# addtt/ladder-vae-pytorch

Measured on AMD Instinct MI355X. Metric: training images/sec (ELBO step: fwd+bwd+Adamax), higher is better.
Workload: dtype f32; 1 GPU; CIFAR10-shaped 15-layer LVAE (BASELINE configs[2]): 32x32x3, zdims 32x15, 4 blocks/layer, 64 filters, gated+skip, DMoL-10, dropout 0.2, free bits 1.0; batch_per_gpu=256, global_batch=256, parallelism=dp1, hip_graph=True

## Files before the change

include/lvae_hip.h:

```cpp
#ifndef LVAE_HIP_H
#define LVAE_HIP_H

#include <stddef.h>
#include <stdint.h>

#ifdef __cplusplus
extern "C" {
#endif

#define LVAE_ABI_VERSION 17

#define LVAE_EINVAL (-1)
#define LVAE_EALIGN (-2)
#define LVAE_EWORKSPACE (-3)

enum { LVAE_STATS_BN_FWD = 0, LVAE_STATS_BN_BWD = 1 };
enum { LVAE_PREC_F32 = 0, LVAE_PREC_BF16 = 1 };
enum { LVAE_DT_F32 = 0, LVAE_DT_BF16 = 1 };
enum {
  LVAE_FORM_AUTO = 0,
  LVAE_FORM_F32_MFMA = 1,
  LVAE_FORM_SIX_PRODUCT = 2,
  LVAE_FORM_SIX_PRODUCT_DIRECT = 3
};
// ... 63 lines not shown
  LVAE_VARIANT_WINO_SIX = 4,
  LVAE_VARIANT_BF16_DIRECT = 5,
  LVAE_VARIANT_SIX_DIRECT = 6
};
int32_t lvae_conv2d_variant(const lvae_conv_desc* d);
int32_t lvae_conv2d_position_major(const lvae_conv_desc* d);
int32_t lvae_resblock_bf16_storage(const lvae_conv_desc* d);
int lvae_conv2d_bf16(const lvae_conv_desc* d, void* stream);
int32_t lvae_conv2d_stats_rows(const lvae_conv_desc* d);
int32_t lvae_conv2d_folds_bn_finalize(const lvae_conv_desc* d);
int32_t lvae_conv2d_stats_buffer_rows(const lvae_conv_desc* d);

size_t lvae_conv2d_prepare_entry_bytes(void);
int lvae_conv2d_prepare_entry(const lvae_conv_desc* d, void* entry);
int lvae_conv2d_prepare_weights(const void* entries, int32_t n, int32_t max_cout, void* stream);

int lvae_conv1x1_gate_f32(const lvae_conv_desc* d, const float* res, int32_t act, float* out, void* stream);
int32_t lvae_conv1x1_gate_stats_rows(const lvae_conv_desc* d);
enum {
  LVAE_GATE_PERSISTENT = 1,
  LVAE_GATE_SINGLE_SHOT = 2
};
int32_t lvae_conv1x1_gate_variant(const lvae_conv_desc* d);
int lvae_conv1x1_gate_bwd_f32(const lvae_conv_desc* d, const float* dout, const float* ab, int32_t act, float* dab,
                              void* stream);
int32_t lvae_conv1x1_gate_bwd_ok(const lvae_conv_desc* d);

typedef struct lvae_bn_apply {
  const float* parts;
  int32_t rows;
  int32_t act;
  int64_t M;
  const float* coef;
  const float* dh;
  const float* x;
  const float* add;
  float* dgamma;
  float* dbeta;
  float* out;
  int32_t dh_bf16;
  int32_t reserved_;
  const float* drop;
} lvae_bn_apply;
size_t lvae_conv1x1_gate_bwd_wgrad_workspace(const lvae_conv_desc* d);
int32_t lvae_conv1x1_gate_bwd_wgrad_apply_ok(const lvae_conv_desc* d);
int lvae_conv1x1_gate_bwd_wgrad_f32(const lvae_conv_desc* d, const float* dout, const float* ab, const float* y, int32_t act,
                                    float* dw, int64_t dw_sk, int64_t dw_sn, float* db, void* workspace, size_t workspace_bytes,
                                    const lvae_bn_apply* ap, void* stream);
int32_t lvae_conv1x1_gate_bwd_wgrad_recompute_ok(const lvae_conv_desc* d);
int lvae_conv1x1_gate_bwd_wgrad_recompute_f32(const lvae_conv_desc* d, const float* dout, const float* y, int32_t act, void* gate_ws,
                                              int64_t gate_ws_bytes, int32_t gate_ws_ready, const float* gate_w, int64_t gate_w_sk,
                                              int64_t gate_w_sn, const float* gate_bias, float* dw, int64_t dw_sk, int64_t dw_sn,
                                              float* db, void* workspace, size_t workspace_bytes, const lvae_bn_apply* ap, void* stream);

enum { LVAE_RB_PRO_AFFINE = 0, LVAE_RB_PRO_BN_APPLY = 1, LVAE_RB_PRO_GATE_BWD = 2 };
enum { LVAE_RB_EPI_PLAIN = 0, LVAE_RB_EPI_GATE = 1 };
typedef struct lvae_rb_ext {
  int32_t prologue, epilogue;
  const float* gate_w;
  int64_t gate_w_sk, gate_w_sn;
  void* gate_ws;
  int64_t gate_ws_bytes;
  int32_t gate_ws_ready;
  const float* gate_bias;
  int32_t act;
  const float* res;
  float* ab;
  float* out;
  float* out_stats;
  const float* out_stats_pivot;
  const float* dout;
  const float* ab_in;
  float* dab;
  const float* bwd_parts;
  int32_t bwd_rows;
  int32_t bwd_act;
  int64_t bwd_M;
  const float* bwd_coef;
  const float* bwd_x;
  float* dgamma;
  float* dbeta;
  const float* pro_drop;
  float* xt_out;
  const void* pf_ptr[2];
  int64_t pf_bytes[2];
  const float* ap_parts;
  int32_t ap_rows;
  int32_t ap_act;
  int64_t ap_M;
  const float* ap_coef;
  const float* ap_dh;
  const float* ap_x;
  const float* ap_add;
  float* ap_dgamma;
  float* ap_dbeta;
  float* ap_out;
} lvae_rb_ext;
size_t lvae_resblock_gate_workspace(const lvae_conv_desc* g);
int lvae_resblock_gate_prepare_entry(const lvae_conv_desc* g, void* entry);
int32_t lvae_resblock_conv_rows(const lvae_conv_desc* d);
int32_t lvae_resblock_conv_gate_rows(const lvae_conv_desc* d);
size_t lvae_resblock_conv_workspace(const lvae_conv_desc* d);
int lvae_resblock_conv_prepare_entry(const lvae_conv_desc* d, void* entry);
int lvae_resblock_conv_f32(const lvae_conv_desc* d, const lvae_rb_ext* ext, void* stream);

size_t lvae_conv2d_wgrad_workspace(const lvae_conv_desc* d);
// ... 257 lines not shown
```

ladder-vae-pytorch_amd/_C.py:

```python
import ctypes as C
import os

import torch

_HERE = os.path.dirname(os.path.abspath(__file__))
LIB_PATH = os.path.join(_HERE, 'liblvae_hip.so')

ACT = {None: 0, 'none': 0, 'elu': 1, 'relu': 2, 'leakyrelu': 3, 'selu': 4}
GATHER_CONV, GATHER_TRANSPOSED = 0, 1
PREC_F32, PREC_BF16 = 0, 1
DT_F32, DT_BF16 = 0, 1
VARIANT_DIRECT, VARIANT_POS, VARIANT_WINO_F32, VARIANT_WINO_SIX, VARIANT_BF16_DIRECT, VARIANT_SIX_DIRECT = 0, 2, 3, 4, 5, 6
GATE_PERSISTENT, GATE_SINGLE_SHOT = 1, 2
WGRAD_VARIANT_GENERIC, WGRAD_VARIANT_IMG, WGRAD_VARIANT_BF16, WGRAD_VARIANT_WINO, WGRAD_VARIANT_DIRECT_1X1, WGRAD_VARIANT_TILE, WGRAD_VARIANT_THIN = range(7)
FEED_U8, FEED_F32 = 0, 1
FORM_AUTO, FORM_F32_MFMA, FORM_SIX_PRODUCT, FORM_SIX_PRODUCT_DIRECT = 0, 1, 2, 3


class LvaeHipError(RuntimeError):
    pass


class ConvDesc(C.Structure):
    _fields_ = [
# ... 47 lines not shown


class LrScheduleStruct(C.Structure):
    _fields_ = [('base_lr', C.c_float), ('min_lr', C.c_float), ('gamma', C.c_float), ('kind', C.c_int32),
                ('warmup_steps', C.c_int64), ('decay_steps', C.c_int64)]


class GradGuardState(C.Structure):
    _fields_ = [('norm', C.c_float), ('scale', C.c_float), ('skip', C.c_int32), ('reserved_', C.c_int32), ('clipped', C.c_uint64),
                ('skipped', C.c_uint64)]


class CopyEntry(C.Structure):
    _fields_ = [('dst', C.c_void_p), ('src', C.c_void_p), ('n', C.c_int64)]


LR_KINDS = {'constant': 0, 'cosine': 1, 'linear': 2, 'step': 3, 'exp': 4}

RB_PRO_AFFINE, RB_PRO_BN_APPLY, RB_PRO_GATE_BWD = 0, 1, 2
RB_EPI_PLAIN, RB_EPI_GATE = 0, 1

ABI_VERSION = 17

_P, _I, _L, _F, _Z, _U = C.c_void_p, C.c_int32, C.c_int64, C.c_float, C.c_size_t, C.c_uint64

SIGNATURES = {
    'lvae_abi_version': (C.c_int, []),
    'lvae_last_error': (C.c_char_p, []),
    'lvae_conv2d_workspace': (_Z, [C.POINTER(ConvDesc)]),
    'lvae_conv2d_f32': (C.c_int, [C.POINTER(ConvDesc), _P]),
    'lvae_conv2d_bf16': (C.c_int, [C.POINTER(ConvDesc), _P]),
    'lvae_conv1x1_dgrad_cat_f32': (C.c_int, [C.POINTER(ConvDesc), _P, _I, _P]),
    'lvae_conv1x1_dgrad_cat_ok': (_I, [C.POINTER(ConvDesc), _I]),
    'lvae_conv2d_stats_rows': (_I, [C.POINTER(ConvDesc)]),
    'lvae_conv2d_variant': (_I, [C.POINTER(ConvDesc)]),
    'lvae_conv2d_position_major': (_I, [C.POINTER(ConvDesc)]),
    'lvae_resblock_bf16_storage': (_I, [C.POINTER(ConvDesc)]),
    'lvae_conv2d_folds_bn_finalize': (_I, [C.POINTER(ConvDesc)]),
    'lvae_conv2d_stats_buffer_rows': (_I, [C.POINTER(ConvDesc)]),
    'lvae_conv2d_prepare_entry_bytes': (_Z, []),
    'lvae_conv2d_prepare_entry': (C.c_int, [C.POINTER(ConvDesc), _P]),
    'lvae_conv2d_prepare_weights': (C.c_int, [_P, _I, _I, _P]),
    'lvae_conv1x1_gate_f32': (C.c_int, [C.POINTER(ConvDesc), _P, _I, _P, _P]),
    'lvae_conv1x1_gate_stats_rows': (_I, [C.POINTER(ConvDesc)]),
    'lvae_conv1x1_gate_variant': (_I, [C.POINTER(ConvDesc)]),
    'lvae_conv1x1_gate_bwd_f32': (C.c_int, [C.POINTER(ConvDesc), _P, _P, _I, _P, _P]),
    'lvae_conv1x1_gate_bwd_ok': (_I, [C.POINTER(ConvDesc)]),
    'lvae_conv1x1_gate_bwd_wgrad_workspace': (_Z, [C.POINTER(ConvDesc)]),
    'lvae_conv1x1_gate_bwd_wgrad_apply_ok': (_I, [C.POINTER(ConvDesc)]),
    'lvae_conv1x1_gate_bwd_wgrad_f32': (C.c_int, [C.POINTER(ConvDesc), _P, _P, _P, _I, _P, _L, _L, _P, _P, _Z, C.POINTER(BnApply), _P]),
    'lvae_conv1x1_gate_bwd_wgrad_recompute_ok': (_I, [C.POINTER(ConvDesc)]),
    'lvae_conv1x1_gate_bwd_wgrad_recompute_f32': (C.c_int, [C.POINTER(ConvDesc), _P, _P, _I, _P, _L, _I, _P, _L, _L, _P, _P, _L, _L, _P, _P, _Z,
                                                            C.POINTER(BnApply), _P]),
    'lvae_resblock_gate_workspace': (_Z, [C.POINTER(ConvDesc)]),
    'lvae_resblock_gate_prepare_entry': (C.c_int, [C.POINTER(ConvDesc), _P]),
    'lvae_resblock_conv_rows': (_I, [C.POINTER(ConvDesc)]),
    'lvae_resblock_conv_gate_rows': (_I, [C.POINTER(ConvDesc)]),
    'lvae_resblock_conv_workspace': (_Z, [C.POINTER(ConvDesc)]),
    'lvae_resblock_conv_prepare_entry': (C.c_int, [C.POINTER(ConvDesc), _P]),
    'lvae_resblock_conv_f32': (C.c_int, [C.POINTER(ConvDesc), C.POINTER(RbExt), _P]),
    'lvae_conv2d_wgrad_workspace': (_Z, [C.POINTER(ConvDesc)]),
    'lvae_conv2d_wgrad_f32': (C.c_int, [C.POINTER(ConvDesc), _P, _P, _P, _P, _Z, _P]),
    'lvae_conv2d_wgrad_bf16': (C.c_int, [C.POINTER(ConvDesc), _P, _P, _P, _P, _Z, _P]),
    'lvae_conv2d_wgrad_variant': (_I, [C.POINTER(ConvDesc)]),
    'lvae_conv2d_wgrad_apply_ok': (_I, [C.POINTER(ConvDesc)]),
    'lvae_conv2d_wgrad_apply_f32': (C.c_int, [C.POINTER(ConvDesc), C.POINTER(BnApply), _P, _P, _P, _Z, _P]),
    'lvae_conv2d_wgrad_pair_ok': (_I, [C.POINTER(ConvDesc), C.POINTER(ConvDesc)]),
    'lvae_conv2d_wgrad_pair_workspace': (_Z, [C.POINTER(ConvDesc), C.POINTER(ConvDesc)]),
    'lvae_conv2d_wgrad_pair_schedule': (_I, [C.POINTER(ConvDesc), C.POINTER(ConvDesc), C.POINTER(_I)]),
    'lvae_conv2d_wgrad_pair_f32': (C.c_int, [C.POINTER(ConvDesc), C.POINTER(BnApply), C.POINTER(ConvDesc), _P, _P, _P, _P, _P, _P, _Z, _P]),
    'lvae_conv2d_wgrad_shared_ok': (_I, [C.POINTER(ConvDesc), _P, _I]),
    'lvae_conv2d_wgrad_shared_workspace': (_Z, [C.POINTER(ConvDesc), _I]),
    'lvae_conv2d_wgrad_shared_schedule': (_I, [C.POINTER(ConvDesc), _P, _I, C.POINTER(_I)]),
    'lvae_conv2d_wgrad_shared_f32': (C.c_int, [C.POINTER(ConvDesc), _P, _P, _P, _I, _P, _Z, _P]),
    'lvae_conv2d_wgrad_grouped_workspace': (_Z, [C.POINTER(ConvDesc), _I]),
    'lvae_conv2d_wgrad_grouped_f32': (C.c_int, [C.POINTER(ConvDesc), _P, _P, _P, _I, _P, _Z, _P]),
    'lvae_conv2d_wgrad_grouped_schedule': (_I, [C.POINTER(ConvDesc), _I, C.POINTER(_I)]),
    'lvae_bn_stats_workspace': (_Z, [_L, _I]),
    'lvae_bn_stats_f32': (C.c_int, [_P, _L, _I, _P, _P, _F, _F, _P, _P, _P, _P, _P, _P, _P, _Z, _P]),
    'lvae_bn_finalize_parts_f32': (C.c_int, [_P, _I, _L, _I, _P, _P, _P, _F, _F, _P, _P, _P, _P, _P, _P, _P]),
    'lvae_bn_eval_coeffs_f32': (C.c_int, [_I, _P, _P, _P, _P, _F, _P, _P, _P]),
    'lvae_affine_act_f32': (C.c_int, [_P, _L, _I, _P, _P, _I, _P, _L, _P, _P]),
    'lvae_affine_act_bwd_f32': (C.c_int, [_P, _P, _L, _I, _P, _P, _I, _I, _P, _P, _P, _P, _P, _L, _P, _P, _P, _Z, _P]),
    'lvae_affine_act_bwd_parts_f32': (C.c_int, [_P, _I, _P, _P, _L, _I, _P, _P, _I, _P, _P, _P, _P, _P, _L, _P, _P, _P, _Z, _I, _P]),
    'lvae_gate_fwd_f32': (C.c_int, [_P, _P, _L, _I, _I, _P, _P]),
    'lvae_gate_bwd_f32': (C.c_int, [_P, _P, _L, _I, _I, _P, _P]),
    'lvae_act_bwd_from_out_f32': (C.c_int, [_P, _P, _L, _I, _P, _P]),
    'lvae_add_f32': (C.c_int, [_P, _P, _L, _P, _P]),
    'lvae_add3_f32': (C.c_int, [_P, _P, _P, _L, _P, _P]),
    'lvae_sum_of_row_means_f32': (C.c_int, [_P, _I, _I, _P, _P]),
    'lvae_scale_rows_add_f32': (C.c_int, [_P, _P, _L, _I, _P, _L, _P, _P]),
    'lvae_colsum_f32': (C.c_int, [_P, _L, _L, _P, _I, _P]),
    'lvae_normal_stochastic_fwd_f32': (C.c_int, [_P, _I, _P, _P, _I, _I, _I, _I, _I, _P, _P, _P, _P, _P, _P]),
    'lvae_normal_stochastic_bwd_f32': (C.c_int, [_P, _I, _P, _P, _P, _P, _P, _P, _P, _P, _I, _I, _I, _I, _I, _P, _P, _P]),
    'lvae_stoch_block_ok': (_I, [C.POINTER(StochBlock)]),
    'lvae_stoch_block_workspace': (_Z, [C.POINTER(ConvDesc)]),
    'lvae_stoch_block_prepare_entry': (C.c_int, [C.POINTER(ConvDesc), _P]),
    'lvae_stoch_block_fwd_f32': (C.c_int, [C.POINTER(StochBlock), _P]),
    'lvae_stoch_block_bwd_ok': (_I, [C.POINTER(StochBlockBwd)]),
    'lvae_stoch_block_bwd_f32': (C.c_int, [C.POINTER(StochBlockBwd), _P]),
    'lvae_normal_prior_sample_f32': (C.c_int, [_P, _I, _P, _F, _P, _I, _I, _I, _P, _P, _P]),
    'lvae_latent_interp_workspace': (_Z, [_I, _I]),
    'lvae_latent_interp_f32': (C.c_int, [_P, _P, _P, _I, _L, _I, _I, _P, _P, _Z, _P]),
    'lvae_kl_elementwise_fwd_f32': (C.c_int, [_P, _I, _P, _I, _P, _I, _I, _I, _I, _P, _P]),
    'lvae_kl_elementwise_bwd_f32': (C.c_int, [_P, _I, _P, _I, _P, _P, _I, _I, _I, _I, _P, _P, _P, _P]),
    'lvae_bernoulli_fwd_f32': (C.c_int, [_P, _P, _P, _I, _L, _P, _P, _P, _P, _P, _P]),
# ... 109 lines not shown
```

ladder-vae-pytorch_amd/kernels.py:

```python
import ctypes as C
import weakref

import torch

from . import _C
from ._C import ACT, BnFold, ConvDesc, RbExt, GATHER_CONV, GATHER_TRANSPOSED, PREC_BF16, PREC_F32, call, ptr, ptr_dt, stream_ptr

_ws_cache = {}

precision = PREC_F32


form = _C.FORM_AUTO


class use_form:
    def __init__(self, f):
        self.f = f

    def __enter__(self):
        global form
        self.prev, form = form, self.f

    def __exit__(self, *exc):
# ... 626 lines not shown
    d_b = _desc(g_b, w_b, x_b, None, N, H, W, H, W, g_b.Cout, g_b.s_ci, g_b.s_co, GATHER_CONV, None, *in_b)
    return d_a, d_b


def conv2d_wgrad_pair_ok(x_a, w_a, g_a, x_b, w_b, g_b):
    ds = _wgrad_pair_descs(x_a, w_a, g_a, x_b, w_b, g_b)
    return ds is not None and bool(_C.load().lvae_conv2d_wgrad_pair_ok(C.byref(ds[0]), C.byref(ds[1])))


def conv2d_wgrad_pair_schedule(x_a, w_a, g_a, x_b, w_b, g_b):
    ds = _wgrad_pair_descs(x_a, w_a, g_a, x_b, w_b, g_b)
    out = (C.c_int32 * 6)()
    if ds is None or not _C.load().lvae_conv2d_wgrad_pair_schedule(C.byref(ds[0]), C.byref(ds[1]), out):
        return None
    return tuple(out[:3]), tuple(out[3:])


def conv2d_wgrad_pair(x, weight, g, dweight, dbias, parts, dh, xbn, coef0, act, dgamma, dbeta, dy_b, weight_b, g_b, dweight_b, dbias_b,
                      drop=None, in_scale=None, in_shift=None, in_act=None, in_scale_b=None, in_shift_b=None, in_act_b=None, out=None):
    _chk_nhwc(x, 'x')
    _chk_nhwc(xbn, 'xbn')
    _chk_nhwc(dy_b, 'dy_b')
    N, H, W, _ = x.shape
    if tuple(dweight.stride()) != tuple(weight.stride()) or tuple(dweight_b.stride()) != tuple(weight_b.stride()):
        raise _C.LvaeHipError("conv2d_wgrad_pair: gradient strides differ from weight strides")
    ds = _wgrad_pair_descs(x, weight, g, xbn, weight_b, g_b, (in_scale, in_shift, in_act), (in_scale_b, in_shift_b, in_act_b))
    if ds is None:
        raise _C.LvaeHipError("conv2d_wgrad_pair: not a pair (fp32 precision, plain convolutions)")
    d_a, d_b = ds
    d_b.y_dtype = _dt(dy_b)
    need = _C.load().lvae_conv2d_wgrad_pair_workspace(C.byref(d_a), C.byref(d_b))
    ws = workspace(need, x.device)
    dy = out if out is not None else torch.empty((N, H, W, g.Cout), dtype=torch.float32, device=x.device)
    ap = _C.BnApply(ptr(parts), parts.shape[0], ACT[act], N * H * W, ptr(coef0), ptr(dh), ptr(xbn), None, ptr(dgamma), ptr(dbeta), ptr(dy), 0, 0, ptr(drop))
    call('lvae_conv2d_wgrad_pair_f32', C.byref(d_a), C.byref(ap), C.byref(d_b), ptr_dt(dy_b), ptr(dweight), ptr(dbias), ptr(dweight_b), ptr(dbias_b),
         ws.data_ptr(), ws.numel(), stream_ptr())
    return dy


def conv1x1_dgrad_cat(dy, weight, g, C1):
    _chk_nhwc(dy, 'dy')
    N, H, W, _ = dy.shape
    if not 0 < C1 < g.Cin:
        return None
    dx = torch.empty((N, H, W, C1), dtype=torch.float32, device=dy.device)
    dx2 = torch.empty((N, H, W, g.Cin - C1), dtype=torch.float32, device=dy.device)
    d = _desc(g, weight, dy, None, N, H, W, H, W, g.Cin, g.s_co, g.s_ci, GATHER_TRANSPOSED, y=dx)
    if not _C.load().lvae_conv1x1_dgrad_cat_ok(C.byref(d), C1):
        return None
    call('lvae_conv1x1_dgrad_cat_f32', C.byref(d), ptr(dx2), C1, stream_ptr())
    return dx, dx2


def conv2d_wgrad(x, dy, weight, g, dweight, dbias=None, x2=None, in_scale=None, in_shift=None, in_act=None):
    _chk_nhwc(x, 'x')
    _chk_nhwc(dy, 'dy')
    N, H, W, _ = x.shape
    OH, OW = dy.shape[1], dy.shape[2]
    if tuple(dweight.stride()) != tuple(weight.stride()):
        raise _C.LvaeHipError("conv2d_wgrad: gradient strides %s differ from weight strides %s" %
                              (tuple(dweight.stride()), tuple(weight.stride())))
    d = _desc(g, weight, x, x2, N, H, W, OH, OW, g.Cout, g.s_ci, g.s_co,
              GATHER_TRANSPOSED if g.transposed else GATHER_CONV, None, in_scale, in_shift, in_act)
    d.y_dtype = _dt(dy)
    need = _C.load().lvae_conv2d_wgrad_workspace(C.byref(d))
    ws = workspace(need, x.device)
    call('lvae_conv2d_wgrad_f32', C.byref(d), ptr_dt(dy), ptr(dweight), ptr(dbias), ws.data_ptr(), ws.numel(), stream_ptr())


def _wgrad_item_arrays(items, who):
    n = len(items)
    descs = (ConvDesc * n)()
    dys, dws, dbs = (C.c_void_p * n)(), (C.c_void_p * n)(), (C.c_void_p * n)()
    for i, (x, dy, weight, g, dweight, dbias, kw) in enumerate(items):
        _chk_nhwc(x, 'x')
        _chk_nhwc(dy, 'dy')
        if tuple(dweight.stride()) != tuple(weight.stride()):
            raise _C.LvaeHipError("%s: gradient strides %s differ from weight strides %s" %
                                  (who, tuple(dweight.stride()), tuple(weight.stride())))
        N, H, W, _ = x.shape
        d = _desc(g, weight, x, kw.get('x2'), N, H, W, dy.shape[1], dy.shape[2], g.Cout, g.s_ci, g.s_co,
                  GATHER_TRANSPOSED if g.transposed else GATHER_CONV, None, kw.get('in_scale'), kw.get('in_shift'), kw.get('in_act'))
        d.y_dtype = _dt(dy)
        C.memmove(C.byref(descs, i * C.sizeof(ConvDesc)), C.byref(d), C.sizeof(ConvDesc))
        dys[i], dws[i], dbs[i] = ptr_dt(dy), ptr(dweight), ptr(dbias)
    return descs, dys, dws, dbs


def _wgrad_shared_descs(convs):
    if precision != PREC_F32 or _ddi is not None or not 1 <= len(convs) <= 3:
        return None
    descs = (ConvDesc * len(convs))()
    for i, (x, weight, g) in enumerate(convs):
        if x.dim() != 4 or x.dtype != torch.float32 or g.transposed:
            return None
        N, H, W, _ = x.shape
        d = _desc(g, weight, x, None, N, H, W, H, W, g.Cout, g.s_ci, g.s_co, GATHER_CONV)
        C.memmove(C.byref(descs, i * C.sizeof(ConvDesc)), C.byref(d), C.sizeof(ConvDesc))
    return descs


def conv2d_wgrad_shared_ok(convs, routed=False):
    descs = _wgrad_shared_descs(convs)
    if descs is None or not _C.load().lvae_conv2d_wgrad_shared_ok(descs, None, len(convs)):
        return False
    if not routed:
# ... 877 lines not shown
```

ladder-vae-pytorch_amd/lib/nn.py:

```python
import math

import torch
from torch import nn
from torch.nn import init

from .. import kernels as K
from .. import ops
from .. import resblock

NONLIN_NAMES = ('relu', 'leakyrelu', 'elu', 'selu')


def act_name(nonlin):
    if isinstance(nonlin, str):
        if nonlin not in NONLIN_NAMES:
            raise KeyError(nonlin)
        return nonlin
    table = {nn.ReLU: 'relu', nn.LeakyReLU: 'leakyrelu', nn.ELU: 'elu', nn.SELU: 'selu'}
    if nonlin in table:
        return table[nonlin]
    raise KeyError(nonlin)


class Placeholder(nn.Module):

    def __init__(self, what=''):
        super().__init__()
        self.what = what

    def extra_repr(self):
        return self.what


class Conv2dParams(nn.Module):

    def __init__(self, c_in, c_out, kernel, stride=1, padding=0, transposed=False, output_padding=0):
        super().__init__()
        self.c_in, self.c_out, self.kernel = c_in, c_out, kernel
        self.stride, self.padding, self.transposed, self.output_padding = stride, padding, transposed, output_padding
        shape = (c_in, c_out, kernel, kernel) if transposed else (c_out, c_in, kernel, kernel)
        self.weight = nn.Parameter(torch.empty(shape))
        self.bias = nn.Parameter(torch.empty(c_out))
        init.kaiming_uniform_(self.weight, a=math.sqrt(5))
        fan_in, _ = init._calculate_fan_in_and_fan_out(self.weight)
        if fan_in != 0:
            bound = 1 / math.sqrt(fan_in)
            init.uniform_(self.bias, -bound, bound)
        self._geom = None
        self._geom_key = None

    def geom(self):
        key = (self.weight.data_ptr(), tuple(self.weight.stride()))
        if self._geom_key != key:
            self._geom = K.ConvGeom(self.weight, self.stride, self.padding, self.transposed, self.output_padding)
            self._geom_key = key
        return self._geom

    def forward(self, x, x2=None, out_act=None):
        return ops.conv(x, self, x2=x2, out_act=out_act)

    def extra_repr(self):
        return '%d->%d k%d s%d p%d%s' % (self.c_in, self.c_out, self.kernel, self.stride, self.padding,
                                          ' transposed' if self.transposed else '')


class BatchNorm2dParams(nn.Module):

    def __init__(self, channels, eps=1e-5, momentum=0.1):
        super().__init__()
        self.eps, self.momentum = eps, momentum
        self.weight = nn.Parameter(torch.ones(channels))
        self.bias = nn.Parameter(torch.zeros(channels))
        self.register_buffer('running_mean', torch.zeros(channels))
        self.register_buffer('running_var', torch.ones(channels))
        self.register_buffer('num_batches_tracked', torch.tensor(0, dtype=torch.long))
        self._pending = 0
        self._register_state_dict_hook(BatchNorm2dParams._flush_hook)

    @staticmethod
    def _flush_hook(module, state_dict, prefix, local_metadata):
        if module._pending:
            module._buffers['num_batches_tracked'] += module._pending
            module._pending = 0
            state_dict[prefix + 'num_batches_tracked'] = module._buffers['num_batches_tracked']

    def note_training_forward(self, n=1):
        self._pending += n


class GateLayer2d(nn.Module):

    def __init__(self, channels, kernel_size, nonlin=nn.LeakyReLU):
        super().__init__()
        assert kernel_size % 2 == 1
        pad = kernel_size // 2
        self.conv = Conv2dParams(channels, 2 * channels, kernel_size, padding=pad)
        self.act = act_name(nonlin)
        self.nonlin = Placeholder(self.act)

    def forward(self, x):
        return ops.GateFn.apply(self.conv(x), None, self.act)

# ... 121 lines not shown
```

ladder-vae-pytorch_amd/ops.py:

```python
from types import SimpleNamespace

import torch
from torch.autograd import Function

from . import kernels as K
from . import resblock as RB

_const_cache = {}


def _ones_zeros(C, device):
    key = (C, device)
    if key not in _const_cache:
        _const_cache[key] = (torch.ones(C, device=device), torch.zeros(C, device=device))
    return _const_cache[key]


def grad_buf(p):
    if not p.requires_grad:
        return None
    if p.grad is None:
        p.grad = torch.zeros_like(p)
    return p.grad

# ... 54 lines not shown
        return K.conv2d_wgrad(x, dy, w, g, dw, db, **kw)
    st = sts[(dw.data_ptr() >> 8) % len(sts)]
    st.wait_stream(torch.cuda.current_stream())
    with torch.cuda.stream(st):
        K.conv2d_wgrad(x, dy, w, g, dw, db, **kw)
    for t in (x, dy, kw.get('x2'), kw.get('in_scale'), kw.get('in_shift')):
        if t is not None:
            t.record_stream(st)


class WgradShare:

    def __init__(self, n_in):
        self.items, self.wait = [], n_in

    @staticmethod
    def plan(convs):
        if not (RB.switches.wgrad_shared and torch.is_grad_enabled() and all(m.weight.requires_grad for _, m in convs)):
            return None
        if not K.conv2d_wgrad_shared_ok([(x, m.weight, m.geom()) for x, m in convs], routed=True):
            return None
        return WgradShare(len(convs) - 1)

    def add(self, item, is_input):
        self.items.append(item)
        self.wait -= int(is_input)
        if self.wait > 0:
            return
        items, self.items = self.items, []
        if (len(items) >= 2 and _side['stream'] is None and all(it[1].dtype == torch.float32 for it in items) and
                K.conv2d_wgrad_shared_ok([(it[0], it[2], it[3]) for it in items])):
            K.conv2d_wgrad_shared(items)
        else:
            for x, dy, w, g, dw, db, kw in items:
                wgrad(x, dy, w, g, dw, db, **kw)


class ConvFn(Function):

    @staticmethod
    def forward(ctx, x, x2, mod, out_act, weight, bias, share=None):
        g = mod.geom()
        y = K.conv2d(x, weight, g, bias=bias, x2=x2, out_act=out_act)
        ctx.mod, ctx.out_act, ctx.g, ctx.share = mod, out_act, g, share
        ctx.has_x2 = x2 is not None
        ctx.save_for_backward(x, x2, y if out_act else None)
        return y

    @staticmethod
    def backward(ctx, dy):
        x, x2, y = ctx.saved_tensors
        mod, g = ctx.mod, ctx.g
        dy = _c(dy)
        if ctx.out_act:
            dy = K.act_bwd_from_out(dy, y, ctx.out_act)
        w = mod.weight
        if w.requires_grad:
            db = grad_buf(mod.bias) if mod.bias is not None else None
            if ctx.share is not None and x2 is None:
                ctx.share[0].add((x, dy, w, g, grad_buf(w), db, {}), ctx.share[1])
            else:
                wgrad(x, dy, w, g, grad_buf(w), db, x2=x2)
        dx = dx2 = None
        hw = (x.shape[1], x.shape[2])
        if x2 is None:
            if ctx.needs_input_grad[0]:
                dx = K.conv2d_dgrad(dy, w, g, hw)
        else:
            C1 = x.shape[3]
            both = K.conv1x1_dgrad_cat(dy, w, g, C1) if (RB.switches.dgrad_cat and ctx.needs_input_grad[0] and ctx.needs_input_grad[1]) else None
            if both is not None:
                dx, dx2 = both
            else:
                if ctx.needs_input_grad[0]:
                    dx = K.conv2d_dgrad(dy, w, g, hw, ci_range=(0, C1))
                if ctx.needs_input_grad[1]:
                    dx2 = K.conv2d_dgrad(dy, w, g, hw, ci_range=(C1, g.Cin))
        return dx, dx2, None, None, None, None, None


def conv(x, mod, x2=None, out_act=None, share=None):
    return ConvFn.apply(x, x2, mod, out_act, mod.weight, mod.bias, share)


def _bn_of_half(h, bn, training, parts, pivot):
    if bn is None:
        return None, _ones_zeros(h.shape[3], h.device) + (None, None)
    if not training:
        return None, K.bn_eval_coeffs(bn.weight, bn.bias, bn.running_mean, bn.running_var, bn.eps) + (None, None)
    if parts is not None:
        return (parts, pivot, bn), None
    return None, K.bn_stats(h, bn.weight, bn.bias, bn.running_mean, bn.running_var, bn.eps, bn.momentum)


def _conv_half(h, bn, cv, act, m, training, parts, pivot, stats_pivot, s16):
    in_bn, coef = _bn_of_half(h, bn, training, parts, pivot)
    if in_bn is not None:
        return K.conv2d(h, cv.weight, cv.geom(), bias=cv.bias, in_act=act, out_scale=m, in_bn=in_bn, stats_pivot=stats_pivot, out_bf16=s16)
    r = K.conv2d(h, cv.weight, cv.geom(), bias=cv.bias, in_scale=coef[0], in_shift=coef[1], in_act=act, out_scale=m, stats_pivot=stats_pivot,
                 out_bf16=s16)
    return (r if stats_pivot is not None else (r, None)) + (coef,)


def _fwd_fused_gate(call, x, blk, m1, m2, training):
    act, st, bn2, cv1, cv2, gate = blk.act, blk.sched, blk.bn2, blk.conv1, blk.conv2, blk.gate
    whole = call.plan.forward == 'whole-image'
    if whole:
        in_bn, coef1 = _bn_of_half(x, blk.bn1, True, call.parts, call.pivot)
        st.link('fwd', K.rb_weight_ranges(x, cv1.weight, cv1.geom(), False))
        y1, parts2, coef1 = K.rb_conv(x, cv1.weight, cv1.geom(), cv1.bias, act, m1, in_bn=in_bn, coef=coef1, stats_pivot=bn2.running_mean,
                                      prefetch=K.rb_weight_ranges(x, cv2.weight, cv2.geom(), False, gate=(gate.weight, gate.geom())))
    else:
        y1, parts2, coef1 = _conv_half(x, blk.bn1, cv1, act, m1, True, call.parts, call.pivot, bn2.running_mean, False)
    in_bn, coef2 = _bn_of_half(y1, bn2, True, parts2, bn2.running_mean)
    call.out_pivot = coef1[2].detach() if call.plan.gate_stats else None
    y2, ab, out, call.out_parts, coef2 = K.rb_conv_gate(y1, cv2.weight, cv2.geom(), cv2.bias, act, m2, gate.weight, gate.geom(), gate.bias, x, act,
                                                        in_bn=in_bn, coef=coef2, stats_pivot=call.out_pivot,
                                                        prefetch=st.next_ranges('fwd') if whole else None,
                                                        want_ab=not call.plan.recompute_ab)
    return y1, y2, ab, out, coef1, coef2


def _fwd_per_op(call, x, blk, m1, m2, training):
    act, bn2, gate, s16 = blk.act, blk.bn2, blk.gate, call.plan.bf16_internals
    want_stats = training and bn2 is not None and bn2.running_mean is not None
    y1, parts2, coef1 = _conv_half(x, blk.bn1, blk.conv1, act, m1, training, call.parts, call.pivot, bn2.running_mean if want_stats else None, s16)
    y2, _, coef2 = _conv_half(y1, bn2, blk.conv2, act, m2, training, parts2, bn2.running_mean if bn2 is not None else None, None, s16)
    if gate is None:
        return y1, y2, None, K.add(y2, x), coef1, coef2
    call.out_pivot = coef1[2].detach() if call.plan.gate_stats else None
    r = K.conv1x1_gate(y2, gate.weight, gate.geom(), gate.bias, x, act, stats_pivot=call.out_pivot)
    ab, out, call.out_parts = r if call.out_pivot is not None else r + (None,)
    return y1, y2, ab, out, coef1, coef2


# ... 593 lines not shown
```

ladder-vae-pytorch_amd/resblock.py:

```python
import os
import weakref
from typing import NamedTuple, Optional

import torch

from . import kernels as K


class Switches:

    def __init__(self, env):
        on = lambda name: env.get(name, '1') != '0'
        self.wgrad_flush = int(env.get('LVAE_WGRAD_FLUSH', '1024'))
        self.dgrad_cat = on('LVAE_DGRAD_CAT')
        self.wgrad_apply = on('LVAE_WGRAD_APPLY')
        self.wgrad_apply_maxw = int(env.get('LVAE_WGRAD_APPLY_MAXW', '16'))
        self.wgrad_pair = on('LVAE_WGRAD_PAIR')
        self.wgrad_pair_maxw = int(env.get('LVAE_WGRAD_PAIR_MAXW', '16'))
        self.wgrad_shared = on('LVAE_WGRAD_SHARED')
        self.gate_stats = env.get('LVAE_NO_GATE_STATS') is None
        self.defer_apply = on('LVAE_DEFER_APPLY')
        self.defer_apply_large = on('LVAE_DEFER_APPLY_LARGE')
        self.rb_fwd_min_hw, self.rb_bwd_min_hw = int(env.get('LVAE_RB_FWD_MIN_HW', '16')), int(env.get('LVAE_RB_BWD_MIN_HW', '1'))
        self.rb_gate_large = on('LVAE_RB_GATE_LARGE')
        self.stoch_block = on('LVAE_STOCH_BLOCK')
        self.stoch_block_bwd = on('LVAE_STOCH_BLOCK_BWD')
        self.gate_recompute = on('LVAE_GATE_RECOMPUTE')
        self.gate_recompute_maxw = int(env.get('LVAE_GATE_RECOMPUTE_MAXW', '16'))


switches = Switches(os.environ)


class BlockPlan(NamedTuple):
    forward: str
    bf16_internals: bool
    gate_stats: bool
    backward: Optional[str]
    wgrad_absorbs_apply: bool
    wgrad_pair: bool
    accepts: Optional[str]
    recompute_ab: bool = False


def plan_block(blk, x, training):
    sw, grad = switches, torch.is_grad_enabled()
    cv1, cv2, gate, bn1, bn2 = blk.conv1, blk.conv2, blk.gate, blk.bn1, blk.bn2
    gated_bn = gate is not None and bn1 is not None and bn2 is not None and gate.bias is not None
    full = (training and gated_bn and cv1.bias is not None and cv2.bias is not None and bn1.running_mean is not None and
            bn2.running_mean is not None and x.dtype == torch.float32)
    hw = x.shape[1] * x.shape[2]
    whole = full and K.rb_rows(x, cv1.weight, cv1.geom()) > 0
    whole_fwd, whole_bwd = whole and 0 < sw.rb_fwd_min_hw <= hw, whole and 0 < sw.rb_bwd_min_hw <= hw
    s16 = bool(not whole_fwd and not whole_bwd and gated_bn and K.resblock_bf16_storage(x, cv1.weight, cv1.geom()))
    if whole_fwd:
        forward = 'whole-image'
    elif full and not s16 and sw.rb_gate_large and K.rb_gate_rows(x, cv2.weight, cv2.geom(), whole_image=False) > 0:
        forward = 'wino-gate'
    else:
        forward = 'per-op' if gate is not None else 'ungated'
    gate_stats = gate is not None and training and bn1 is not None and bn1.running_mean is not None and sw.gate_stats
    backward, accepts, absorbs, pair = None, None, False, False
    if grad and whole_bwd:
        backward, accepts = 'whole-image', 'f32-dh'
    elif grad:
        backward = 'composed'
        if gate is not None and gate.bias is not None and gate.weight.requires_grad and \
                K.gate_bwd_fused_ws(x, gate.weight, gate.geom(), gate.weight.grad) > 0:
            backward = 'persistent-gate'
            if training and not whole_fwd and sw.defer_apply_large and K.gate_bwd_apply_ok(x, gate.weight, gate.geom(), gate.weight.grad):
                accepts = 'any-dh'
        absorbs = bool(training and bn2 is not None and sw.wgrad_apply and not s16 and cv1.weight.requires_grad and
# ... 68 lines not shown
```

Baseline: 9349 images/s.

## Fuse 1x1 concat-conv backward dgrad, wgrad and deferred BN apply into one kernel

```diff
diff --git a/include/lvae_hip.h b/include/lvae_hip.h
--- a/include/lvae_hip.h
+++ b/include/lvae_hip.h
@@ -139,6 +139,11 @@
                                               int64_t gate_ws_bytes, int32_t gate_ws_ready, const float* gate_w, int64_t gate_w_sk,
                                               int64_t gate_w_sn, const float* gate_bias, float* dw, int64_t dw_sk, int64_t dw_sn,
                                               float* db, void* workspace, size_t workspace_bytes, const lvae_bn_apply* ap, void* stream);
+
+size_t lvae_conv1x1_cat_bwd_workspace(const lvae_conv_desc* d, int32_t split);
+int32_t lvae_conv1x1_cat_bwd_apply_ok(const lvae_conv_desc* d, int32_t split);
+int lvae_conv1x1_cat_bwd_f32(const lvae_conv_desc* d, const float* x1, const float* x2, float* dx1, float* dx2, float* dweight, float* dbias,
+                             const lvae_bn_apply* ap, void* workspace, size_t workspace_bytes, int32_t max_workgroups, void* stream);
 
 enum { LVAE_RB_PRO_AFFINE = 0, LVAE_RB_PRO_BN_APPLY = 1, LVAE_RB_PRO_GATE_BWD = 2 };
 enum { LVAE_RB_EPI_PLAIN = 0, LVAE_RB_EPI_GATE = 1 };
diff --git a/ladder-vae-pytorch_amd/_C.py b/ladder-vae-pytorch_amd/_C.py
--- a/ladder-vae-pytorch_amd/_C.py
+++ b/ladder-vae-pytorch_amd/_C.py
@@ -123,6 +123,9 @@
     'lvae_conv1x1_gate_bwd_wgrad_recompute_ok': (_I, [C.POINTER(ConvDesc)]),
     'lvae_conv1x1_gate_bwd_wgrad_recompute_f32': (C.c_int, [C.POINTER(ConvDesc), _P, _P, _I, _P, _L, _I, _P, _L, _L, _P, _P, _L, _L, _P, _P, _Z,
                                                             C.POINTER(BnApply), _P]),
+    'lvae_conv1x1_cat_bwd_workspace': (_Z, [C.POINTER(ConvDesc), _I]),
+    'lvae_conv1x1_cat_bwd_apply_ok': (_I, [C.POINTER(ConvDesc), _I]),
+    'lvae_conv1x1_cat_bwd_f32': (C.c_int, [C.POINTER(ConvDesc), _P, _P, _P, _P, _P, _P, C.POINTER(BnApply), _P, _Z, _I, _P]),
     'lvae_resblock_gate_workspace': (_Z, [C.POINTER(ConvDesc)]),
     'lvae_resblock_gate_prepare_entry': (C.c_int, [C.POINTER(ConvDesc), _P]),
     'lvae_resblock_conv_rows': (_I, [C.POINTER(ConvDesc)]),
diff --git a/ladder-vae-pytorch_amd/csrc/conv1x1_cat_bwd_fused.hip b/ladder-vae-pytorch_amd/csrc/conv1x1_cat_bwd_fused.hip
--- /dev/null
+++ b/ladder-vae-pytorch_amd/csrc/conv1x1_cat_bwd_fused.hip
@@ -0,0 +1,342 @@
+#include "bf16_frag.h"
+#include "bn_stats.h"
+#include "lvae_host.h"
+
+namespace lvae {
+
+struct CbfArgs {
+  const float* dy;
+  const float* x1;
+  const float* x2;
+  const float* w;
+  int64_t w_sn;
+  float* dx1;
+  float* dx2;
+  float* slab_w;
+  float* slab_b;
+  int M, ntiles;
+  lvae_bn_apply ap;
+};
+
+constexpr int CB_LDD = 72;
+constexpr int CB_LDX = 136;
+constexpr int CB_LDO = 128;
+constexpr size_t cbf_lds() {
+  return (size_t)3 * (64 * CB_LDD + 64 * CB_LDX) * 2 + (size_t)64 * CB_LDO * 4 + 6 * 64 * 4 + (size_t)4 * 4 * 3 * 64 * 16;
+}
+static_assert(cbf_lds() <= 160 * 1024, "one workgroup's LDS");
+
+__device__ __forceinline__ int cb_swz(int row) { return ((row >> 2) & 1) << 5; }
+
+template <bool AP>
+__global__ __launch_bounds__(512) void conv1x1_cat_bwd_fused_kernel(CbfArgs a) {
+  kernarg_warmup<sizeof(CbfArgs)>();
+  extern __shared__ __attribute__((aligned(16))) unsigned char smem_raw[];
+  constexpr int D_PLANE = 64 * CB_LDD, X_PLANE = 64 * CB_LDX;
+  __bf16* Ds = reinterpret_cast<__bf16*>(smem_raw);
+  __bf16* Xs = Ds + 3 * D_PLANE;
+  float* Os = reinterpret_cast<float*>(Xs + 3 * X_PLANE);
+  float* Cf = Os + 64 * CB_LDO;
+  bf16x8* Wf = reinterpret_cast<bf16x8*>(Cf + 6 * 64);
+  const int t = threadIdx.x, lane = t & 63, wave = t >> 6;
+  const bool wg_role = wave >= 4;
+  const int wm = (wave & 3) >> 1, wn = wave & 1, li = lane & 31, lh = lane >> 5, G = lane >> 4, i16 = lane & 15;
+  const f32x4 zero4 = {0.f, 0.f, 0.f, 0.f};
+
+  if (AP) {
+    const int q = t & 31, rg = t >> 5, rows = a.ap.rows;
+    f32x4 acc = zero4;
+    for (int r = rg; r < rows; r += 16 * 8) {
+      f32x4 v[8];
+#pragma unroll
+      for (int u = 0; u < 8; ++u) {
+        const int rr = r + 16 * u;
+        v[u] = *reinterpret_cast<const f32x4*>(a.ap.parts + (size_t)(rr < rows ? rr : 0) * 128 + q * 4);
+      }
+#pragma unroll
+      for (int u = 0; u < 8; ++u)
+        if (r + 16 * u < rows) acc += v[u];
+    }
+    *reinterpret_cast<f32x4*>(Os + rg * 128 + q * 4) = acc;
+    if (t < 256) Cf[t] = a.ap.coef[t];
+    __syncthreads();
+    if (t < 64) {
+      double sa = 0.0, sb = 0.0;
+#pragma unroll
+      for (int g = 0; g < 16; ++g) {
+        sa += (double)Os[g * 128 + t];
+        sb += (double)Os[g * 128 + 64 + t];
+      }
+      const BnBwdChannel r = bn_bwd_finish(sa, sb, a.ap.M);
+      Cf[256 + t] = r.c1;
+      Cf[320 + t] = r.c2;
+      if (blockIdx.x == 0) {
+        if (a.ap.dbeta) a.ap.dbeta[t] += r.dbeta;
+        if (a.ap.dgamma) a.ap.dgamma[t] += r.dgamma;
+      }
+    }
+    __syncthreads();
+  }
+  auto ap_value = [&](const f32x4 dh, const f32x4 xv, const f32x4 ad, int c) {
+    const f32x4 sc = *reinterpret_cast<const f32x4*>(Cf + c), sh = *reinterpret_cast<const f32x4*>(Cf + 64 + c);
+    const f32x4 mu = *reinterpret_cast<const f32x4*>(Cf + 128 + c), rs = *reinterpret_cast<const f32x4*>(Cf + 192 + c);
+    const f32x4 c1 = *reinterpret_cast<const f32x4*>(Cf + 256 + c), c2 = *reinterpret_cast<const f32x4*>(Cf + 320 + c);
+    const f32x4 g = dh * act_grad4(xv * sc + sh, a.ap.act);
+    return bn_bwd_apply(g, xv, c1, c2, mu, rs, sc) + ad;
+  };
+
+  if (!wg_role) {
+    const int cb = wave;
+#pragma unroll
+    for (int s = 0; s < 4; ++s) {
+      const float* wp = a.w + (int64_t)(cb * 32 + li) * a.w_sn + 16 * s + 8 * lh;
+      bf16x8 v[3];
+      split_frag<3>(*reinterpret_cast<const f32x4*>(wp), *reinterpret_cast<const f32x4*>(wp + 4), v);
+#pragma unroll
+      for (int q = 0; q < 3; ++q) Wf[((s * 4 + cb) * 3 + q) * 64 + lane] = v[q];
+    }
+  }
+
+  f32x4 pg[2], p1[2], p2[2];
+  f32x4 px[AP ? 2 : 1], pd[AP ? 2 : 1];
+  const int c4 = (t & 15) * 4, r0 = t >> 4;
+  const bool ap_add = AP && a.ap.add != nullptr, ap_out = AP && a.ap.out != nullptr;
+  auto prefetch_row = [&](int tile, int u) {
+    const int m = tile * 64 + r0 + 32 * u;
+    const size_t mc = m < a.M ? (size_t)m : 0;
+    if (AP) {
+      pg[u] = *reinterpret_cast<const f32x4*>(a.ap.dh + mc * 64 + c4);
+      px[u] = *reinterpret_cast<const f32x4*>(a.ap.x + mc * 64 + c4);
+      pd[u] = ap_add ? *reinterpret_cast<const f32x4*>(a.ap.add + mc * 64 + c4) : zero4;
+    } else {
+      pg[u] = *reinterpret_cast<const f32x4*>(a.dy + mc * 64 + c4);
+    }
+    p1[u] = *reinterpret_cast<const f32x4*>(a.x1 + mc * 64 + c4);
+    p2[u] = *reinterpret_cast<const f32x4*>(a.x2 + mc * 64 + c4);
+  };
+
+  f32x16 accw[2];
+#pragma unroll
+  for (int j = 0; j < 2; ++j)
+#pragma unroll
+    for (int r = 0; r < 16; ++r) accw[j][r] = 0.f;
+  f32x4 bs = zero4;
+  const int trow = 8 * (G >> 1) + (i16 >> 2), tch = 16 * (G & 1) + 4 * (i16 & 3);
+  using PO = PieceOrder<3>;
+
+  int tile = blockIdx.x;
+  if (tile < a.ntiles) {
+    prefetch_row(tile, 0);
+    prefetch_row(tile, 1);
+  }
+  for (; tile < a.ntiles; tile += gridDim.x) {
+    const int m0 = tile * 64;
+    const bool more = tile + (int)gridDim.x < a.ntiles;
+    f32x4 g[2], v1[2], v2[2];
+#pragma unroll
+    for (int u = 0; u < 2; ++u) {
+      g[u] = v1[u] = v2[u] = zero4;
+      if (m0 + r0 + 32 * u < a.M) {
+        g[u] = AP ? ap_value(pg[u], px[u], pd[u], c4) : pg[u];
+        v1[u] = p1[u];
+        v2[u] = p2[u];
+      }
+      if (more) prefetch_row(tile + gridDim.x, u);
+    }
+#pragma unroll
+    for (int u = 0; u < 2; ++u) {
+      const int r = r0 + 32 * u;
+      if (ap_out && m0 + r < a.M) store_wt4(a.ap.out + (size_t)(m0 + r) * 64 + c4, g[u]);
+      bs += g[u];
+      bf16x4 qg[3], q1[3], q2[3];
+      split4<3>(g[u], qg);
+      split4<3>(v1[u], q1);
+      split4<3>(v2[u], q2);
+#pragma unroll
+      for (int q = 0; q < 3; ++q) {
+        *reinterpret_cast<bf16x4*>(Ds + q * D_PLANE + r * CB_LDD + c4) = qg[q];
+        *reinterpret_cast<bf16x4*>(Xs + q * X_PLANE + r * CB_LDX + c4) = q1[q];
+        *reinterpret_cast<bf16x4*>(Xs + q * X_PLANE + r * CB_LDX + 64 + c4) = q2[q];
+      }
+    }
+    lds_barrier();
+
+    if (!wg_role) {
+      f32x16 accx[2];
+#pragma unroll
+      for (int j = 0; j < 2; ++j)
+#pragma unroll
+        for (int r = 0; r < 16; ++r) accx[j][r] = 0.f;
+#pragma unroll
+      for (int s = 0; s < 4; ++s) {
+        bf16x8 af[3];
+#pragma unroll
+        for (int q = 0; q < 3; ++q) af[q] = *reinterpret_cast<const bf16x8*>(Ds + q * D_PLANE + (wm * 32 + li) * CB_LDD + 16 * s + 8 * lh);
+#pragma unroll
+        for (int j = 0; j < 2; ++j) {
+          bf16x8 bw[3];
+#pragma unroll
+          for (int q = 0; q < 3; ++q) bw[q] = Wf[((s * 4 + wn * 2 + j) * 3 + q) * 64 + lane];
+#pragma unroll
+          for (int k = 0; k < PO::N; ++k) accx[j] = __builtin_amdgcn_mfma_f32_32x32x16_bf16(af[PO::A[k]], bw[PO::B[k]], accx[j], 0, 0, 0);
+        }
+      }
+#pragma unroll
+      for (int j = 0; j < 2; ++j)
+#pragma unroll
+        for (int r = 0; r < 16; ++r) {
+          const int row = wm * 32 + (r & 3) + 8 * (r >> 2) + 4 * lh;
+          Os[row * CB_LDO + (((wn * 2 + j) * 32 + li) ^ cb_swz(row))] = accx[j][r];
+        }
+    } else {
+#pragma unroll
+      for (int s = 0; s < 4; ++s) {
+        bf16x8 bf[3];
+#pragma unroll
+        for (int q = 0; q < 3; ++q) {
+          const __bf16* dp = Ds + q * D_PLANE + (16 * s + trow) * CB_LDD + wn * 32 + tch;
+          bf[q] = tr_frag(dp, dp + 4 * CB_LDD);
+        }
+#pragma unroll
+        for (int j = 0; j < 2; ++j) {
+          bf16x8 af[3];
+#pragma unroll
+          for (int q = 0; q < 3; ++q) {
+            const __bf16* xp = Xs + q * X_PLANE + (16 * s + trow) * CB_LDX + (wm * 2 + j) * 32 + tch;
+            af[q] = tr_frag(xp, xp + 4 * CB_LDX);
+          }
+#pragma unroll
+          for (int k = 0; k < PO::N; ++k) accw[j] = __builtin_amdgcn_mfma_f32_32x32x16_bf16(af[PO::A[k]], bf[PO::B[k]], accw[j], 0, 0, 0);
+        }
+      }
+    }
+    lds_barrier();
+#pragma unroll
+    for (int u = 0; u < 2; ++u) {
+      const int r = r0 + 32 * u, m = m0 + r;
+      if (m < a.M) {
+        const f32x4 lo = *reinterpret_cast<const f32x4*>(Os + r * CB_LDO + (c4 ^ cb_swz(r)));
+        const f32x4 hi = *reinterpret_cast<const f32x4*>(Os + r * CB_LDO + ((64 + c4) ^ cb_swz(r)));
+        store_wt4(a.dx1 + (size_t)m * 64 + c4, lo);
+        store_wt4(a.dx2 + (size_t)m * 64 + c4, hi);
+      }
+    }
+  }
+
+  float* sw = a.slab_w + (size_t)blockIdx.x * 128 * 64;
+  if (wg_role) {
+#pragma unroll
+    for (int j = 0; j < 2; ++j)
+#pragma unroll
+      for (int r = 0; r < 16; ++r)
+        sw[(size_t)((wm * 2 + j) * 32 + (r & 3) + 8 * (r >> 2) + 4 * lh) * 64 + wn * 32 + li] = accw[j][r];
+  }
+  if (a.slab_b) {
+    __syncthreads();
+    float* red = Os;
+    *reinterpret_cast<f32x4*>(red + r0 * 64 + c4) = bs;
+    __syncthreads();
+    if (t < 64) {
+      float v = 0.f;
+#pragma unroll
+      for (int gq = 0; gq < 32; ++gq) v += red[gq * 64 + t];
+      a.slab_b[(size_t)blockIdx.x * 64 + t] = v;
+    }
+  }
+}
+
+static int cbf_nwg(int64_t M, int max_workgroups) {
+  const int64_t ntiles = (M + 63) / 64;
+  const int64_t cap = max_workgroups > 0 && max_workgroups < 256 ? max_workgroups : 256;
+  return (int)(ntiles < cap ? ntiles : cap);
+}
+
+static bool conv1x1_cat_bwd_plan(const lvae_conv_desc* d, int split, bool with_apply, ConvPlan& p) {
+  static const bool off = tune("LVAE_DISABLE_CAT_BWD_FUSED", 0) != 0;
+  (void)with_apply;
+  if (off || d == nullptr) return false;
+  if (d->KH != 1 || d->KW != 1 || d->stride != 1 || d->pad != 0 || d->OH != d->H || d->OW != d->W) return false;
+  if (d->C1 != 64 || d->C2 != 0 || d->x2 != nullptr || d->Cout != 128 || split != 64) return false;
+  if (d->w == nullptr || d->w_sk != 1 || d->w_sn < 64 || d->w_sn % 4 != 0 || !al16_or_null(d->w) || !al16_or_null(d->x)) return false;
+  if (d->bias != nullptr || d->in_scale != nullptr || d->in_shift != nullptr || d->out_scale != nullptr || d->stats_out != nullptr) return false;
+  if (d->in_act != 0 || d->out_act != 0 || d->in_fold != nullptr) return false;
+  if (d->precision != LVAE_PREC_F32 || d->form == LVAE_FORM_F32_MFMA) return false;
+  if (d->x_dtype != LVAE_DT_F32 || d->y_dtype != LVAE_DT_F32) return false;
+  if (d->N <= 0 || d->H <= 0 || d->W <= 0) return false;
+  const int64_t M = (int64_t)d->N * d->H * d->W;
+  if (M >= ((int64_t)1 << 31) - 64) return false;
+  p = ConvPlan{};
+  p.workspace = (size_t)cbf_nwg(M, 0) * (128 * 64 + 64) * sizeof(float);
+  return true;
+}
+
+}
+
+using namespace lvae;
+
+extern "C" size_t lvae_conv1x1_cat_bwd_workspace(const lvae_conv_desc* d, int32_t split) {
+  ConvPlan p;
+  return conv1x1_cat_bwd_plan(d, split, false, p) ? p.workspace : 0;
+}
+
+extern "C" int32_t lvae_conv1x1_cat_bwd_apply_ok(const lvae_conv_desc* d, int32_t split) {
+  ConvPlan p;
+  return conv1x1_cat_bwd_plan(d, split, true, p) ? 1 : 0;
+}
+
+#define CBF_REQUIRE_AL16(p) LVAE_REQUIRE(al16_or_null(p), LVAE_EALIGN, "lvae_conv1x1_cat_bwd_f32: " #p " must be 16-byte aligned")
+
+extern "C" int lvae_conv1x1_cat_bwd_f32(const lvae_conv_desc* d, const float* x1, const float* x2, float* dx1, float* dx2, float* dweight,
+                                        float* dbias, const lvae_bn_apply* ap, void* workspace, size_t workspace_bytes,
+                                        int32_t max_workgroups, void* stream) {
+  const char* who = "lvae_conv1x1_cat_bwd_f32";
+  const bool with_ap = ap != nullptr && ap->parts != nullptr;
+  LVAE_REQUIRE(d && (d->x || with_ap) && x1 && x2 && dx1 && dx2 && dweight && workspace, LVAE_EINVAL, "%s: null pointer", who);
+  LVAE_REQUIRE(max_workgroups >= 0, LVAE_EINVAL, "%s: negative max_workgroups", who);
+  ConvPlan p;
+  LVAE_REQUIRE(conv1x1_cat_bwd_plan(d, 64, with_ap, p), LVAE_EINVAL,
+               "%s: not taken (needs the dgrad view of a 1x1 / stride-1 convolution over a 64 + 64 channel concat with 64 output channels: "
+               "C1 = 64, Cout = 128, w_sk = 1, 16-byte aligned dy and w, fp32 tensors, precision LVAE_PREC_F32 and not LVAE_FORM_F32_MFMA); "
+               "use lvae_conv2d_wgrad_f32 + lvae_conv1x1_dgrad_cat_f32", who);
+  if (with_ap)
+    LVAE_REQUIRE(ap->rows > 0 && ap->M == (int64_t)d->N * d->H * d->W && ap->coef && ap->dh && ap->x && ap->dh_bf16 == 0 && ap->drop == nullptr,
+                 LVAE_EINVAL, "%s: deferred apply needs parts / rows, M = N*H*W, the coefficient block, an fp32 dh and x, and no drop", who);
+  LVAE_REQUIRE(workspace_bytes >= p.workspace, LVAE_EWORKSPACE, "%s: workspace %zu < %zu", who, workspace_bytes, p.workspace);
+  CBF_REQUIRE_AL16(x1);
+  CBF_REQUIRE_AL16(x2);
+  CBF_REQUIRE_AL16(dx1);
+  CBF_REQUIRE_AL16(dx2);
+  CBF_REQUIRE_AL16(workspace);
+  CbfArgs a;
+  a.ap = lvae_bn_apply{};
+  if (with_ap) {
+    CBF_REQUIRE_AL16(ap->parts);
+    CBF_REQUIRE_AL16(ap->coef);
+    CBF_REQUIRE_AL16(ap->dh);
+    CBF_REQUIRE_AL16(ap->x);
+    CBF_REQUIRE_AL16(ap->add);
+    CBF_REQUIRE_AL16(ap->out);
+    a.ap = *ap;
+  }
+  a.dy = d->x;
+  a.x1 = x1;
+  a.x2 = x2;
+  a.w = d->w;
+  a.w_sn = d->w_sn;
+  a.dx1 = dx1;
+  a.dx2 = dx2;
+  a.M = d->N * d->H * d->W;
+  a.ntiles = (a.M + 63) / 64;
+  const int nwg = cbf_nwg(a.M, max_workgroups);
+  a.slab_w = static_cast<float*>(workspace);
+  a.slab_b = dbias ? a.slab_w + (size_t)nwg * 128 * 64 : nullptr;
+  constexpr size_t lds = cbf_lds();
+  const dim3 grid(nwg), block(512);
+  hipStream_t s = (hipStream_t)stream;
+  const int rc = with_ap ? launch_lds<conv1x1_cat_bwd_fused_kernel<true>>(who, grid, block, lds, (int)lds, s, a)
+                         : launch_lds<conv1x1_cat_bwd_fused_kernel<false>>(who, grid, block, lds, (int)lds, s, a);
+  if (rc) return rc;
+  wgrad_reduce_launch(a.slab_w, a.slab_b, nwg, 1, 128, 64, 0, d->w_sn, d->w_sk, dweight, dbias, s);
+  LVAE_LAUNCH_CHECK("lvae_conv1x1_cat_bwd_f32 reduce");
+  return 0;
+}
diff --git a/ladder-vae-pytorch_amd/kernels.py b/ladder-vae-pytorch_amd/kernels.py
--- a/ladder-vae-pytorch_amd/kernels.py
+++ b/ladder-vae-pytorch_amd/kernels.py
@@ -702,6 +702,52 @@
     return dx, dx2
 
 
+def _cat_bwd_desc(dy_like, weight, g, C1, dweight):
+    if _ddi is not None or dy_like.dim() != 4 or g.transposed or dy_like.dtype != torch.float32 or not 0 < C1 < g.Cin:
+        return None
+    if dweight is not None and tuple(dweight.stride()) != tuple(weight.stride()):
+        return None
+    N, H, W, _ = dy_like.shape
+    return _desc(g, weight, dy_like, None, N, H, W, H, W, g.Cin, g.s_co, g.s_ci, GATHER_TRANSPOSED)
+
+
+def cat_bwd_ws(dy_like, weight, g, C1, dweight=None):
+    d = _cat_bwd_desc(dy_like, weight, g, C1, dweight)
+    return int(_C.load().lvae_conv1x1_cat_bwd_workspace(C.byref(d), C1)) if d is not None else 0
+
+
+def cat_bwd_apply_ok(dy_like, weight, g, C1, dweight=None):
+    d = _cat_bwd_desc(dy_like, weight, g, C1, dweight)
+    return d is not None and bool(_C.load().lvae_conv1x1_cat_bwd_apply_ok(C.byref(d), C1))
+
+
+def conv1x1_cat_bwd(dy, x, x2, weight, g, dweight, dbias, apply=None, store_dy=False, max_workgroups=0, scratch=None):
+    _chk_nhwc(dy, 'dy')
+    C1 = x.shape[3]
+    d = _cat_bwd_desc(dy, weight, g, C1, dweight)
+    if d is None or x.dtype != torch.float32 or x2 is None or x2.dtype != torch.float32 or tuple(x.shape[:3]) != tuple(dy.shape[:3]) or \
+            tuple(x2.shape[:3]) != tuple(dy.shape[:3]) or x2.shape[3] != g.Cin - C1 or not (x.is_contiguous() and x2.is_contiguous()):
+        return None
+    lib = _C.load()
+    need = lib.lvae_conv1x1_cat_bwd_workspace(C.byref(d), C1)
+    if not need or (apply is not None and (not lib.lvae_conv1x1_cat_bwd_apply_ok(C.byref(d), C1) or apply.dh.dtype != torch.float32)):
+        return None
+    ws = scratch if scratch is not None else workspace(need, dy.device)
+    if ws.numel() < need or ws.data_ptr() % 16 or any(t is not None and t.data_ptr() % 16 for t in (x, x2)):
+        return None
+    N, H, W, _ = dy.shape
+    ap = None
+    if apply is not None:
+        d.x = None
+        ap = _C.BnApply(ptr(apply.parts), apply.parts.shape[0], ACT[apply.act], N * H * W, ptr(apply.coef0), ptr(apply.dh), ptr(apply.x),
+                        ptr(apply.add), ptr(apply.dgamma), ptr(apply.dbeta), ptr(apply.out) if store_dy else None, 0, 0)
+    dx = torch.empty((N, H, W, C1), dtype=torch.float32, device=dy.device)
+    dx2 = torch.empty((N, H, W, g.Cin - C1), dtype=torch.float32, device=dy.device)
+    call('lvae_conv1x1_cat_bwd_f32', C.byref(d), ptr(x), ptr(x2), ptr(dx), ptr(dx2), ptr(dweight), ptr(dbias),
+         C.byref(ap) if ap is not None else None, ws.data_ptr(), ws.numel(), int(max_workgroups), stream_ptr())
+    return dx, dx2
+
+
 def conv2d_wgrad(x, dy, weight, g, dweight, dbias=None, x2=None, in_scale=None, in_shift=None, in_act=None):
     _chk_nhwc(x, 'x')
     _chk_nhwc(dy, 'dy')
diff --git a/ladder-vae-pytorch_amd/lib/nn.py b/ladder-vae-pytorch_amd/lib/nn.py
--- a/ladder-vae-pytorch_amd/lib/nn.py
+++ b/ladder-vae-pytorch_amd/lib/nn.py
@@ -48,6 +48,7 @@
             init.uniform_(self.bias, -bound, bound)
         self._geom = None
         self._geom_key = None
+        self.__dict__['sched'] = resblock.BlockState()
 
     def geom(self):
         key = (self.weight.data_ptr(), tuple(self.weight.stride()))
diff --git a/ladder-vae-pytorch_amd/ops.py b/ladder-vae-pytorch_amd/ops.py
--- a/ladder-vae-pytorch_amd/ops.py
+++ b/ladder-vae-pytorch_amd/ops.py
@@ -130,9 +130,22 @@
         x, x2, y = ctx.saved_tensors
         mod, g = ctx.mod, ctx.g
         dy = _c(dy)
+        w = mod.weight
+        if x2 is not None:
+            st = getattr(mod, 'sched', None)
+            pend = st.take_pending(dy) if st is not None else None
+            if (RB.switches.merge_bwd_fused and not ctx.out_act and w.requires_grad and ctx.needs_input_grad[0] and ctx.needs_input_grad[1] and
+                    _side['stream'] is None and dy.dtype == torch.float32 and
+                    dy.shape[0] * dy.shape[1] * dy.shape[2] >= RB.switches.merge_bwd_min_rows):
+                both = K.conv1x1_cat_bwd(dy, x, x2, w, g, grad_buf(w), grad_buf(mod.bias) if mod.bias is not None else None, apply=pend)
+                if both is not None:
+                    return both + (None,) * 5
+            if pend is not None:
+                C = pend.coef0.numel()
+                sc, sh, mean, rstd = torch.as_strided(pend.coef0, (4, C), (C, 1)).unbind(0)
+                K.affine_act_bwd_parts(pend.parts, pend.dh, pend.x, sc, sh, pend.act, mean, rstd, pend.dgamma, pend.dbeta, add=pend.add, out=pend.out)
         if ctx.out_act:
             dy = K.act_bwd_from_out(dy, y, ctx.out_act)
-        w = mod.weight
         if w.requires_grad:
             db = grad_buf(mod.bias) if mod.bias is not None else None
             if ctx.share is not None and x2 is None:
@@ -157,8 +170,25 @@
         return dx, dx2, None, None, None, None, None
 
 
+def merge_announces(x, x2, mod, y, out_act):
+    sw = RB.switches
+    if not (sw.merge_bwd_fused and x2 is not None and out_act is None and mod.training and torch.is_grad_enabled()):
+        return False
+    if not (mod.weight.requires_grad and x.requires_grad and x2.requires_grad and y.dtype == torch.float32):
+        return False
+    if y.shape[0] * y.shape[1] * y.shape[2] < sw.merge_bwd_min_rows:
+        return False
+    return K.cat_bwd_apply_ok(y, mod.weight, mod.geom(), x.shape[3], mod.weight.grad)
+
+
 def conv(x, mod, x2=None, out_act=None, share=None):
-    return ConvFn.apply(x, x2, mod, out_act, mod.weight, mod.bias, share)
+    st = getattr(mod, 'sched', None)
+    if st is not None:
+        st.pending = None
+    y = ConvFn.apply(x, x2, mod, out_act, mod.weight, mod.bias, share)
+    if st is not None and merge_announces(x, x2, mod, y, out_act):
+        y._lvae_handover = RB.Handover(None, None, st, 'any-dh')
+    return y
 
 
 def _bn_of_half(h, bn, training, parts, pivot):
diff --git a/ladder-vae-pytorch_amd/resblock.py b/ladder-vae-pytorch_amd/resblock.py
--- a/ladder-vae-pytorch_amd/resblock.py
+++ b/ladder-vae-pytorch_amd/resblock.py
@@ -18,6 +18,8 @@
         self.wgrad_pair = on('LVAE_WGRAD_PAIR')
         self.wgrad_pair_maxw = int(env.get('LVAE_WGRAD_PAIR_MAXW', '16'))
         self.wgrad_shared = on('LVAE_WGRAD_SHARED')
+        self.merge_bwd_fused = on('LVAE_MERGE_BWD_FUSED')
+        self.merge_bwd_min_rows = int(env.get('LVAE_MERGE_BWD_MIN_ROWS', '65536'))
         self.gate_stats = env.get('LVAE_NO_GATE_STATS') is None
         self.defer_apply = on('LVAE_DEFER_APPLY')
         self.defer_apply_large = on('LVAE_DEFER_APPLY_LARGE')
```

Result: faster. 9475 images/s (median of 6 runs) (+1.3%).
